# yeyupiaoling/PPASR

Measured on AMD Instinct MI355X. Metric: audio-seconds/s (RTF^-1) Conformer-streaming fbank, batch32 per GPU, ctc_greedy, higher is better.
Workload: dtype f32; 1 GPU; configs[1]: Conformer streaming (configs/conformer.yml), fbank-80, 32 x 10 s utterances per GPU, V=4233, ctc_greedy, features resident in HBM -> token ids + scores on device; global_batch=32, frames=1000, decoder=ctc_greedy, parallelism=utterance-dp1, pipelined=False, gemm=f32

## Files before the change

### ppasr_amd/csrc/capi.hip

```cpp
#include <cxxabi.h>
#include <cstdlib>

#include "capi_internal.h"

namespace ppasr {
thread_local LaunchProf g_launch_prof;
}

static thread_local std::string g_err;
std::string& ppasr_err_slot() { return g_err; }


ppasr_status upload_pe_table(ppasr_model_s* m, BlobMap& sd, const float** pe_dev) {
  const int d = m->desc.output_size > 0 ? m->desc.output_size : kD;
  const int max_len = m->desc.max_len > 0 ? m->desc.max_len : 5000;
  m->desc.max_len = max_len;
  std::vector<float> pe((size_t)max_len * d);
  auto it = sd.find("__pe_table__");
  if (it != sd.end() && it->second.numel() == pe.size()) {
    std::memcpy(pe.data(), it->second.p, pe.size() * sizeof(float));
  } else {
    for (int i = 0; i < d / 2; ++i) {
      float div = expf((float)(2 * i) * (float)(-(std::log(10000.0) / d)));
      for (int pos = 0; pos < max_len; ++pos) {
// ... 290 lines not shown
      }
      const float* ws[3] = {wq, wk, wv};
      UP4(pack_b(d, 3 * d, [&](int k, int n) { return ws[n / d][(size_t)k * d + (n % d)]; }), L.wqkv);
      std::vector<float> bqkv(3 * d);
      std::memcpy(&bqkv[0], bq, d * sizeof(float));
      std::memcpy(&bqkv[d], bk, d * sizeof(float));
      std::memcpy(&bqkv[2 * d], bv, d * sizeof(float));
      UP(bqkv, L.bqkv);
      UP4(pack_b(d, d, [&](int k, int n) { return wo[(size_t)k * d + n]; }), L.wo);
      UP(vec_of(bo, d), L.bo);
      if (rel) {
        UP(vec_of(pu, pbn), L.pos_u);
        UP(vec_of(pv, pbn), L.pos_v);
        const float* bpos_dev = nullptr;
        if (bp) UP(vec_of(bp, d), bpos_dev);
        const float* wpos_dev = nullptr;
        UP(vec_of(wp, (size_t)d * d), wpos_dev);
        void* pt = nullptr;
        HIP_TRY(hipMalloc(&pt, (size_t)max_len * d * sizeof(float)));
        m->allocs.push_back(pt);
        launch_posproj(pe_dev, wpos_dev, bpos_dev, static_cast<float*>(pt), max_len, nullptr, d);
        HIP_TRY(hipGetLastError());
        L.ptab = static_cast<const float*>(pt);
      } else {
        L.pos_u = L.pos_v = L.ptab = m->zero_vec;
      }
      if (go.concat_after) {
        GET(wc, p + "concat_linear.weight", (size_t)2 * d * d);
        GET(bc, p + "concat_linear.bias", d);
        UP4(pack_b(2 * d, d, [&](int k, int n) { return wc[(size_t)k * d + n]; }), m->gen_x[i].wcat);
        UP(vec_of(bc, d), m->gen_x[i].bcat);
      }
    }
    if (go.use_cnn) {
      GET(p1w, p + "conv_module.pointwise_conv1.weight", 2 * d * d);
      GET(p1b, p + "conv_module.pointwise_conv1.bias", 2 * d);
      GET(dww, p + "conv_module.depthwise_conv.weight", d * KSi);
      GET(dwb, p + "conv_module.depthwise_conv.bias", d);
      GET(p2w, p + "conv_module.pointwise_conv2.weight", d * d);
      GET(p2b, p + "conv_module.pointwise_conv2.bias", d);
      UP4(pack_b(d, 2 * d, [&](int k, int n) { return p1w[(size_t)n * d + k]; }), L.pw1);
      std::vector<float> b1p(p1b, p1b + 2 * d), gp(d);
      for (int c = 0; c < d; ++c) gp[c] = p1b[c] * (1.0f / (1.0f + expf(-p1b[c + d])));
      UP(b1p, L.pw1_b);
      UP(gp, L.glu_pad);
      std::vector<float> dwt((size_t)KSi * d);
// ... 464 lines not shown
    bt_off += (n + 15) / 16 * 16;
    p.tab = t;
    return p;
  };
  int Ti = Tp, mul = sub, pstride = 1;
  bool s1_done = false;
  for (int i = 0; i < h->desc.num_blocks; ++i) {
    const LayerW& L = h->layers[i];
    const int Mi = B * Ti;
    const int grp = h->layer_group[i];
    auto fusable = [&](int layer) {
      return h->layer_group[layer] == 1 && h->desc.attention_heads == 4 && !h->taps && fuse_rows(Mi);
    };
    const PadSkip ps = pskip(Ti, mul);
    const int rows = (!h->taps && conv_ffn_16_supported(h->layer_ks[i], Ti)) ? row_block_for(h, B, Ti, mul, ps.slack, skip) : 32;
    const bool r16 = rows == 16 && h->ffn_split < 0;
    const bool fuse_attn = !r16 && fusable(i);
    const int S = r16 ? 1 : ffn_split_for(h, Mi);
    const bool w16 = rows == kW16 && S == 1;
    const PadSkip psb = S == 1 ? with_table(ps, Ti, r16 ? 16 : 32) : ps;
    const bool h3 = h->gemm_mode == PPASR_GEMM_F16X3 && !h->layers_h3.empty() && !r16 && !w16 && S == 1;
    const bool h3s = h->gemm_mode == PPASR_GEMM_F16X3 && !h->layers_h3.empty() && S > 1;
    const LayerW& Lk = (h3 || h3s) ? h->layers_h3[i] : L;
    auto vt_for = [&](bool fused, bool mode) {
      VtOut v = fused ? vt_out : VtOut{};
      v.k_h3 = (fused && mode) ? 1 : 0;
      return v;
    };
    float* partial = y1;
    float* x3 = ctx;
    if (!s1_done) {
      if (S > 1) {
        timed(3, [&] {
          launch_ffn_split(xa, L.ln_mac_g, L.ln_mac_b, Lk.ffm_w1, L.ffm_b1, Lk.ffm_w2, L.ffm_b2, 0.5f, nullptr, nullptr, partial,
                           xb, Mi, n_chunks, S, st, ps, false, h3s);
          launch_ln_qkv(xb, qkv, Lk, Mi, st, ps, nullptr, nullptr, h3s);
        });
      } else if (r16) {
        timed(3, [&] { launch_ffn_qkv_16(xa, xb, qkv, L, Mi, n_chunks, st, psb); });
      } else if (w16) {
        timed(3, [&] { launch_ffn_qkv_w16(xa, xb, qkv, L, Mi, n_chunks, st, psb, fuse_attn ? vt_out : VtOut{}); });
      } else {
        timed(3, [&] { launch_ffn_qkv(xa, xb, qkv, Lk, Mi, n_chunks, st, psb, vt_for(fuse_attn, h3), h3); });
      }
    }
    s1_done = false;
    tap(xb, (size_t)Mi * kD);
    tap(qkv, (size_t)Mi * 3 * kD);
    const int Tt = (Ti + grp - 1) / grp;
    AttnArgs a{qkv, 768, qkv + 256, 768, qkv + 512, 768, Tt, Tt, 0, lens, ctx, L.pos_u, L.pos_v, (h3 && fuse_attn) ? Lk.ptab : L.ptab, pstride,
               mul * grp, Ti, Ti, grp};
    a.pad_skip = skip ? ps.slack + 1 : 0;
    a.vt = vt_out.vt;
    a.vt_stride = vt_out.stride;
    if (fuse_attn) {
      timed(9, [&] { launch_attn_out_glu(a, B, xb, xc, g, Lk, st, h3); });
    } else {
      timed(4, [&] { launch_attention(a, B, h->desc.attention_heads, st); });
      tap(ctx, (size_t)Mi * kD);
      if (r16) timed(5, [&] { launch_out_glu_16(ctx, xb, xc, g, L, lens, Mi, Ti, mul, st, psb); });
      else if (w16) timed(5, [&] { launch_out_glu_w16(ctx, xb, xc, g, L, lens, Mi, Ti, mul, st, psb); });
      else timed(5, [&] { launch_out_glu(ctx, xb, xc, g, nullptr, h3s ? Lk : L, lens, Mi, Ti, mul, st, psb, S > 1 ? xa : nullptr, h3s); });
    }
    tap(xc, (size_t)Mi * kD);
    tap(g, (size_t)Mi * kD);
    if (eff && i == h->desc.stride_layer_idx) {
      const int Ts = (Ti + 1) / 2;
      timed(6, [&] {
        const int Ss = r16 ? 1 : ffn_split_for(h, B * Ts);
        if (Ss > 1) {
          launch_conv_ffn_stride(g, nullptr, xc, xa, h3s ? Lk : L, lens, B, Ti, Ts, n_chunks, h->layer_ks[i], mul * 2, st,
                                 pskip(Ts, mul * 2), h->desc.causal != 0, h3s, ctx);
          launch_ffn_split(ctx, L.ln_ff_g, L.ln_ff_b, Lk.ff_w1, L.ff_b1, Lk.ff_w2, L.ff_b2, 0.5f, L.ln_fin_g, L.ln_fin_b, partial,
                           xa, B * Ts, n_chunks, Ss, st, pskip(Ts, mul * 2), false, h3s);
        } else {
          launch_conv_ffn_stride(g, nullptr, xc, xa, (h3 || h3s) ? Lk : L, lens, B, Ti, Ts, n_chunks, h->layer_ks[i], mul * 2, st,
                                 pskip(Ts, mul * 2), h->desc.causal != 0, h3 || h3s);
        }
      });
      Ti = Ts;
      mul *= 2;
      pstride *= 2;
    } else if (S > 1) {
      timed(6, [&] {
        launch_conv_pre(g, nullptr, xc, x3, Lk, lens, Mi, Ti, h->layer_ks[i], mul, st, h->desc.causal != 0, ps, h3s);
        launch_ffn_split(x3, L.ln_ff_g, L.ln_ff_b, Lk.ff_w1, L.ff_b1, Lk.ff_w2, L.ff_b2, 0.5f, L.ln_fin_g, L.ln_fin_b, partial,
                         xa, Mi, n_chunks, S, st, ps, false, h3s);
      });
    } else {
      const LayerW* next = (i + 1 < h->desc.num_blocks) ? (h3 ? &h->layers_h3[i + 1] : &h->layers[i + 1]) : nullptr;
      timed(next ? 8 : 6, [&] {
        if (r16)
          launch_conv_ffn_16(g, xc, next ? nullptr : xa, L, lens, Mi, Ti, n_chunks, h->layer_ks[i], mul, next, xb, qkv, st,
                             h->desc.causal != 0, psb);
        else if (w16)
          launch_conv_ffn_w16(g, xc, next ? nullptr : xa, L, lens, Mi, Ti, n_chunks, h->layer_ks[i], mul, next, xb, qkv, st,
                              h->desc.causal != 0, psb, (next && fusable(i + 1)) ? vt_out : VtOut{});
        else
          launch_conv_ffn(g, nullptr, xc, (next && !h->taps) ? nullptr : xa, Lk, lens, Mi, Ti, n_chunks, h->layer_ks[i], mul,
                          next, xb, qkv, st, h->desc.causal != 0, psb,
                          vt_for(next && fusable(i + 1), h3), h3);
      });
      s1_done = next != nullptr;
    }
    tap(xa, (size_t)B * Ti * kD);
  }
  const int Mo = B * Ti;
  float* lg = logits ? logits : probs;
  int32_t* fa = frame_argmax ? frame_argmax : reinterpret_cast<int32_t*>(ws + wl.fa);
  float* fp = frame_maxprob ? frame_maxprob : ws + wl.fp;
  timed(7, [&] {
    const bool head_h3 = h->gemm_mode == PPASR_GEMM_F16X3 && h->head_w_h3;
    HeadW hw = h->head;
    if (head_h3) hw.w = h->head_w_h3;
    launch_ctc_head(xa, hw, lg, fa, fp, ws + wl.rmax, ws + wl.rsum, Mo, st, pskip(Ti, mul),
                    wide_slices_for(h, Mo, std::min((hw.n_tiles + 7) / 8, 32)), y1, head_h3);
  });
  if (probs) {
    if (logits)
      HIP_TRY(hipMemcpyAsync(probs, logits, (size_t)Mo * h->head.V * sizeof(float), hipMemcpyDeviceToDevice, st));
    launch_softmax_from_stats(probs, ws + wl.rmax, ws + wl.rsum, Mo, h->head.V, st, pskip(Ti, mul));
  }
  if (skip) launch_zero_pad_rows(probs, logits, fa, fp, lens, B, Ti, mul, h->head.V, st);
  HIP_TRY(hipGetLastError());
// ... 617 lines not shown
```

### ppasr_amd/csrc/conformer_kernels.h

```cpp
#pragma once
#include <hip/hip_runtime.h>
#include <stdint.h>

#include "rowblock.h"

namespace ppasr {

struct LayerW {
  const float *ln_mac_g, *ln_mac_b, *ln_mha_g, *ln_mha_b, *ln_conv_g, *ln_conv_b;
  const float *ln_ff_g, *ln_ff_b, *ln_fin_g, *ln_fin_b, *ln_cm_g, *ln_cm_b;
  float cm_eps;
  const f32x4 *ffm_w1, *ffm_w2, *ff_w1, *ff_w2, *wqkv, *wo, *pw1, *pw2;
  const float *ffm_b1, *ffm_b2, *ff_b1, *ff_b2, *bqkv, *bo, *pw1_b, *pw2_b;
  const float *dw_w;
  const float *dw_b;
  const float *glu_pad;
  const float *pos_u, *pos_v;
  const float *ptab;
};

struct FrontW {
  const float *cmvn_mean, *cmvn_istd;
  const float *conv1_w, *conv1_b;
  const f32x4 *conv2_w;
  const f32x4 *conv2_wp = nullptr;
  const float *conv2_b;
  int conv2_k = 3, conv2_s = 2;
  const f32x4 *conv3_w = nullptr;
  const float *conv3_b = nullptr;
  const f32x4 *embed_w;
  const float *embed_b;
};

struct HeadW {
  const float *ln_g, *ln_b;
  const f32x4 *w;
  const float *b;
  int V, n_tiles;
};

struct SessDesc {
// ... 6 lines not shown
struct AttnArgs {
  const float* q;
  int q_stride;
  const float* k;
  int k_stride;
  const float* v;
  int v_stride;
  int T1, T2;
  int pos0;
  const int64_t* lens;
  float* ctx;
  const float *pos_u, *pos_v;
  const float* ptab;
  int pos_stride;
  int mask_mul;
  int q_frames, kv_frames;
  int group;
  const SessDesc* sess;
  long long sess_stride;
  int pad_skip;
  const float* vt = nullptr;
  int vt_stride = 0;
  int dm = 256;
};
struct VtOut {
  float* vt = nullptr;
  int stride = 0;
  int k_h3 = 0;
};

constexpr size_t kLdsExclusive = 82 * 1024;
size_t ragged_lds(size_t lds, const PadSkip& ps, int n_blocks);

bool launch_attention_t(const AttnArgs& a, int B, int H, hipStream_t st);
hipError_t configure_attention_kernels();

void launch_block_table(const PadSkip& ps, int M, int R, int* tab, hipStream_t st);

bool conv2_quad_supported(const FrontW& fw);
bool conv12_supported(const FrontW& fw, int F, int F2);
void launch_conv12(const float* feats, const FrontW& fw, float* y2, int B, int T, int F, int Tp, int F2, hipStream_t st,
                   const PadSkip& ps_frames, int* tile_scratch);
void launch_conv2_quad(const float* y1, const FrontW& fw, float* y2, int B, int T1, int F1, int Tp, int F2, hipStream_t st,
                       const PadSkip& ps_frames, int* tile_scratch);
hipError_t configure_front_fused_kernels();

void launch_ffn_qkv_16(const float* x_in, float* x1, float* qkv, const LayerW& w, int M, int n_chunks, hipStream_t st,
                       const PadSkip& ps);
void launch_out_glu_16(const float* ctx, const float* x1, float* x2, float* g, const LayerW& w, const int64_t* lens, int M,
                       int Tp, int mask_mul, hipStream_t st, const PadSkip& ps);
void launch_out_glu_split_16(const float* ctx, const float* x1, float* x2, float* g, float* xhat, const LayerW& w,
// ... 1 lines not shown
                             float* hist = nullptr, int lo = 0);
void launch_shift_caches(float* kc, float* vc, long long layer_stride, int D, int n_layers, int from_full, int keep_full,
                         int from_half, int keep_half, unsigned long long half_mask, hipStream_t st);
void launch_oproj_ln_16(const float* ctx, const float* x1, float* x2_sink, float* xhat_out, const LayerW& w, int M,
                        hipStream_t st, const PadSkip& ps = PadSkip{});
void launch_pw1_glu_cols_16(const float* x, float* g, const LayerW& w, int M, hipStream_t st, float* hist = nullptr, int lo = 0,
                            const float* hist_scale = nullptr, const float* hist_bias = nullptr, const PadSkip& ps = PadSkip{},
                            const int64_t* lens = nullptr, int Tp = 1, int mask_mul = 1);
bool conv_ffn_16_supported(int ksize, int Tp);
void launch_conv_ffn_16(const float* g, const float* x2, float* x_out, const LayerW& w, const int64_t* lens, int M, int Tp,
                        int n_chunks, int ksize, int mask_mul, const LayerW* next, float* x1_next, float* qkv_next,
                        hipStream_t st, bool causal, const PadSkip& ps);
void launch_ffn_qkv_w16(const float* x_in, float* x1, float* qkv, const LayerW& w, int M, int n_chunks, hipStream_t st,
                        const PadSkip& ps, VtOut vt);
void launch_out_glu_w16(const float* ctx, const float* x1, float* x2, float* g, const LayerW& w, const int64_t* lens, int M,
                        int Tp, int mask_mul, hipStream_t st, const PadSkip& ps);
void launch_conv_ffn_w16(const float* g, const float* x2, float* x_out, const LayerW& w, const int64_t* lens, int M, int Tp,
                         int n_chunks, int ksize, int mask_mul, const LayerW* next, float* x1_next, float* qkv_next,
                         hipStream_t st, bool causal, const PadSkip& ps, VtOut vt_next);
hipError_t configure_conformer_t_kernels();

void launch_posproj(const float* pe, const float* wpos , const float* bpos_or_null, float* ptab,
                    int max_len, hipStream_t st, int d = 256);
void launch_conv1(const float* feats, const FrontW& fw, float* y1, int B, int T, int F, int T1, int F1, hipStream_t st,
                  const PadSkip& ps = PadSkip{}, int channels = 256);
void launch_conv_stage(const float* y_in, const f32x4* w, const float* bias, float* y_out, int B, int T_in, int F_in,
                       int T_out, int F_out, int k, int s, hipStream_t st, const PadSkip& ps_frames = PadSkip{},
                       int channels = 256, int* tile_scratch = nullptr,
                       bool h3 = false,
                       float* part = nullptr, size_t part_floats = 0);
size_t conv_stage_part_floats(int M, int channels = 256);
size_t conv_stage_part_reserve(int M);
void launch_conv2(const float* y1, const FrontW& fw, float* y2, int B, int T1, int F1, int Tp, int F2, hipStream_t st,
                  const PadSkip& ps = PadSkip{}, int* tile_scratch = nullptr, const f32x4* w_h3 = nullptr, float* part = nullptr,
                  size_t part_floats = 0);
void launch_embed(const float* y2, const FrontW& fw, float* x0, int M, int K, float xscale, bool scale_before_bias,
                  hipStream_t st, const PadSkip& ps = PadSkip{}, int k_slices = 1, float* part = nullptr,
                  const f32x4* w_h3 = nullptr);
void launch_dense(const float* a, int lda, const f32x4* w, const float* bias, float* out, int M, int K, int n_cols_padded,
                  int ldc, int n_valid, hipStream_t st, float scale = 1.0f, float* part = nullptr, size_t part_floats = 0);
void launch_ffn_qkv(const float* x_in, float* x1, float* qkv, const LayerW& w, int M, int n_chunks, hipStream_t st,
                    const PadSkip& ps = PadSkip{}, VtOut vt = VtOut{}, bool h3 = false);
void launch_repack_h3(const f32x4* src, f32x4* dst, int n_tiles, int G, unsigned int* ovf, hipStream_t st);
inline bool conv_ffn_h3_supported(int ksize) { return ksize == 15 || ksize == 7; }
void launch_split_rows_h3(const float* src, float* dst, long long n_rows, unsigned int* ovf, hipStream_t st);
unsigned int* conformer_h3_ovf_counter();
// ... 87 lines not shown
```

### ppasr_amd/csrc/conformer_kernels.hip

```cpp
#include <cstdlib>

#include "conformer_kernels.h"
#include "launch.h"
#include "phases.h"
#include "h3.h"

#include <math.h>

namespace ppasr {
#ifdef PPASR_PHASE_TS
}
extern "C" __attribute__((visibility("default"))) int ppasr_debug_read_phase_ts(long long* out) {
  return (int)hipMemcpyFromSymbol(out, HIP_SYMBOL(ppasr::g_phase_ts), sizeof(long long) * 128);
}
extern "C" __attribute__((visibility("default"))) int ppasr_debug_read_wave_ts(long long* out) {
  return (int)hipMemcpyFromSymbol(out, HIP_SYMBOL(ppasr::g_wave_ts), sizeof(long long) * 512);
}
extern "C" __attribute__((visibility("default"))) int ppasr_debug_read_wg_ts(long long* out) {
  return (int)hipMemcpyFromSymbol(out, HIP_SYMBOL(ppasr::g_wg_ts), sizeof(long long) * 2 * 1024);
}
namespace ppasr {
#endif


// ... 40 lines not shown

template <bool H3 = false>
__device__ __forceinline__ void ffn_qkv_body(float* bufX, float* bufA, float* bufH, float* __restrict__ x1,
                                             float* __restrict__ qkv, const LayerW& w, int r0, int valid, int n_chunks,
                                             BRing<1>& ring, VtOut vt = VtOut{}) {
  const int lane = lane_id(), wave = wave_id();
  rb_layernorm(bufX, bufA, kLda, kRows, w.ln_mac_g, w.ln_mac_b, 1e-5f);
  __syncthreads();
  PPASR_TS(8);
  f32x16 acc2[1][1];
  acc_zero(acc2);
  const f32x4* wq = w.wqkv + (size_t)wave * kTs256;
  if constexpr (H3) ffn_phase_h3(bufA, w.ffm_w1, w.ffm_b1, w.ffm_w2, n_chunks, wq, ring, acc2);
  else ffn_phase<true>(bufA, bufH, w.ffm_w1, w.ffm_b1, w.ffm_w2, n_chunks, wq, ring, acc2);
  PPASR_TS(9);
  residual_epilogue_t(bufX, acc2, w.ffm_b2, 0.5f);
  __syncthreads();
  PPASR_TS(10);
  rb_store_rows(x1 + (size_t)r0 * kD, bufX, kLda, kRows, valid);
  rb_layernorm(bufX, bufA, kLda, kRows, w.ln_mha_g, w.ln_mha_b, 1e-5f);
  __syncthreads();
  if constexpr (H3) h3_planes_from_tile(bufA, reinterpret_cast<_Float16*>(bufA));
  PPASR_TS(11);
  f32x16 tile[3][1][1];
  bool qk_bad = false;
  const int cq = wave * 32 + 4 * (lane >> 5);
  float* qrow = (lane & 31) < valid ? qkv + (size_t)(r0 + (lane & 31)) * 768 + cq : nullptr;
  f32x4 qb[2][4];
#pragma unroll
  for (int c = 0; c < 2; ++c)
#pragma unroll
    for (int q = 0; q < 4; ++q) qb[c][q] = *reinterpret_cast<const f32x4*>(w.bqkv + c * 256 + cq + 8 * q);
#pragma unroll
  for (int c = 0; c < 3; ++c) {
    acc_zero(tile[c]);
    const f32x4* seg = w.wqkv + (size_t)(c * 8 + wave) * kTs256;
    const f32x4* nseg = c < 2 ? seg + 8 * kTs256 : nullptr;
    if constexpr (H3) {
      const _Float16* pa = reinterpret_cast<const _Float16*>(bufA);
      if (c < 2)
        rb_gemm_h3(pa, seg, nseg, ring, tile[c][0][0]);
      else
        rb_gemm_h3_rows<1, 16, QkStoreTailH3>(pa, kLdh, kPlaneH, seg, nseg, ring, tile[c],
                                              QkStoreTailH3{tile[0][0][0], tile[1][0][0], qrow, qb, vt.k_h3 != 0, qk_bad, cq});
    } else if (c == 0) {
      rb_gemm<1, 1, kG256, kPF, NoSide, true>(bufA, kLda, seg, 0, nseg, 0, ring, tile[c]);
    } else if (c == 1) {
      rb_gemm<1, 1, kG256, kPF, QkvStoreSide, true>(bufA, kLda, seg, 0, nseg, 0, ring, tile[c],
                                                    QkvStoreSide{tile[0][0][0], qrow, qb[0]});
    } else {
      rb_gemm<1, 1, kG256, kPF, QkvStoreSide, false>(bufA, kLda, seg, 0, nseg, 0, ring, tile[c],
                                                     QkvStoreSide{tile[1][0][0], qrow ? qrow + 256 : nullptr, qb[1]});
    }
    PPASR_TS(12 + c);
  }
  if constexpr (H3) h3_note(qk_bad);
  if (vt.vt) {
    const float bv = w.bqkv[2 * 256 + wave * 32 + (lane & 31)];
    float* dst = vt.vt + ((size_t)wave * (vt.stride >> 3) + (r0 >> 3)) * 256 + 4 * lane;
    if constexpr (H3) tile[2][0][0] *= kH3Inv;
#pragma unroll
    for (int i = 0; i < 4; ++i) {
      const f32x16& t = tile[2][0][0];
      *reinterpret_cast<f32x4*>(dst + i * 256) = f32x4{t[4 * i] + bv, t[4 * i + 1] + bv, t[4 * i + 2] + bv, t[4 * i + 3] + bv};
    }
  } else {
    const int col = 2 * 256 + wave * 32 + (lane & 31);
    const float bv = w.bqkv[col];
    if constexpr (H3) tile[2][0][0] *= kH3Inv;
#pragma unroll
    for (int r = 0; r < 16; ++r) {
      int row = acc_row(r, lane);
      if (row < valid) qkv[(size_t)(r0 + row) * 768 + col] = tile[2][0][0][r] + bv;
    }
  }
}
// ... 212 lines not shown
    launch_out_glu_split_16(ctx, x1, x2, g, xh, w, lens, M, Tp, mask_mul, st, ps, move ? hm->hist : nullptr, move ? hm->lo : 0);
    if (move) hm->done = true;
    return;
  }
  const dim3 grid((M + kRows - 1) / kRows);
  if (h3)
    PPASR_LAUNCH(k_out_glu<true>, grid, dim3(kThreads), kLdsOutGlu + 512, st, ctx, x1, x2, g, xh, w, lens, M, Tp, mask_mul, ps,
                 split_xhat ? 1 : 0);
  else
    PPASR_LAUNCH(k_out_glu<false>, grid, dim3(kThreads), kLdsOutGlu, st, ctx, x1, x2, g, xh, w, lens, M, Tp, mask_mul, ps,
                 split_xhat ? 1 : 0);
  if (split_xhat) {
    if (h3)
      PPASR_LAUNCH(k_pw1_glu_cols<true>, dim3(grid.x, 2), dim3(kThreads), kLdsPw1Cols + 512, st, xh, g, w, M, ps);
    else
      PPASR_LAUNCH(k_pw1_glu_cols<false>, dim3(grid.x, 2), dim3(kThreads), kLdsPw1Cols, st, xh, g, w, M, ps);
  }
}

constexpr int kPLd = 68;
constexpr int kPTile = 32 * kPLd;
constexpr int kFusedAttnFloats = kWaves * kPTile + kWaves * 64 + kRows * kLda;
static_assert(2 * kRows * kLda <= kWaves * kPTile + kWaves * 64, "bufX/bufA alias the attention scratch");
static_assert(kRows * kLda + 128 + 4 * kPTile <= kWaves * kPTile, "Q'_v (fp16 x3: its planes, 512 B longer) and the four merge tiles fit in front of Stat");
static_assert(kH3TileBytes <= kRows * kLda * 4 + 512, "fp16 x3: the Q'_u planes at bufC run 512 B past it (the launch asks for them)");
static_assert(kRows * kLda * 4 + kH3TileBytes <= kWaves * kPTile * 4, "fp16 x3: operand planes at bufA stay in front of Stat");
static_assert(kFusedAttnFloats * 4 <= 160 * 1024, "LDS budget");
template <bool H3>
__device__ __forceinline__ void attn_out_glu_body(const AttnArgs& a, int B, const float* __restrict__ x1, float* __restrict__ x2,
                                                  float* __restrict__ g, const LayerW& w) {
  extern __shared__ __attribute__((aligned(16))) float smem[];
  float* Ps = smem;
  float* Stat = Ps + kWaves * kPTile;
  float* bufC = Stat + kWaves * 64;
  float* bufX = smem;
  float* bufA = bufX + kRows * kLda;
  const int lane = lane_id(), wave = wave_id();
  const int h = wave >> 1, khalf = wave & 1;
  const int nq = (a.T1 + 31) / 32;
  const int slot = blockIdx.x >> 3;
  const int b = (slot / nq) * 8 + (blockIdx.x & 7);
  const int q0 = (slot % nq) * 32;
  if (b >= B) return;
  const int T = a.T1;
  const int valid = min(32, T - q0);
  const float* __restrict__ qb = a.q + (size_t)b * T * a.q_stride;
  const float* __restrict__ kbp = a.k + (size_t)b * a.T2 * a.k_stride;
  const float* __restrict__ vbp = a.v + (size_t)b * a.T2 * a.v_stride;
  const float* __restrict__ ptab = a.ptab + (size_t)a.pos0 * kD;
  const int pstride = a.pos_stride;
  const int64_t len_b = a.lens ? a.lens[b] : (int64_t)a.mask_mul * a.T2;
  int T2 = a.T2;
  if (a.pad_skip > 0 && a.lens) {
    const int64_t lb = len_b > 0 ? len_b : 0;
    const int64_t n_valid = (lb + a.mask_mul - 1) / a.mask_mul;
    if (q0 >= min((int64_t)T, n_valid + (a.pad_skip - 1))) return;
    T2 = (int)max((int64_t)1, min((int64_t)T2, n_valid));
  }
  float* QV = Ps;
  float* P = Ps + kRows * kLda + (H3 ? 128 : 0) + (wave >> 1) * kPTile;
  BRing<1> ring;
  const f32x4* seg_o = w.wo + (size_t)wave * kTs256;
  const f32x4* seg_val = w.pw1 + (size_t)wave * kTs256;
  const f32x4* seg_gate = w.pw1 + (size_t)(8 + wave) * kTs256;
  const int hh = lane >> 5, l31 = lane & 31;
  constexpr int NG = 16, PF = 4;
  PPASR_TS(32);
  PPASR_WG_TS(512 + 0);

  const int mrow0 = b * T;
  const int shift = mrow0 & 7;
  int kv_end = (int)min((int64_t)T2, max((int64_t)0, (len_b + a.mask_mul - 1) / a.mask_mul));
  const int U = kv_end > 0 ? kv_end + shift : 0;
  constexpr float kScale = 0.125f * 1.4426950408889634f * (H3 ? 1.0f / (kH3Sa * kH3Sa) : 1.0f);
  const __amdgpu_buffer_rsrc_t rs_k = wstream_rsrc(kbp + h * (H3 ? 32 : 64)), rs_p = wstream_rsrc(ptab + h * (H3 ? 32 : 64)),
                               rs_v = wstream_rsrc(a.vt + ((size_t)(2 * h) * (a.vt_stride >> 3) + ((mrow0 - shift) >> 3)) * 256);
  const int voff_v = lane * 16;
  const int kstride_b = a.k_stride * 4, pstride_b = pstride * kD * 4;
  int vk[2], vp[2];
  auto key_offsets = [&](int u0) {
#pragma unroll
    for (int t = 0; t < 2; ++t) {
      const int key = min(max(u0 - shift + 32 * t + l31, 0), kv_end - 1);
      vk[t] = key * kstride_b + 16 * hh;
      vp[t] = key * pstride_b + 16 * hh;
    }
  };
  auto kfrag = [&](int t, int gk) -> f32x4 {
    return gk < 8 ? wstream_load(rs_k, vk[t], gk * 32) : wstream_load(rs_p, vp[t], (gk - 8) * 32);
  };
  constexpr int NKB = H3 ? 4 : 2;
  f32x4 kq[NKB][4][2];
  auto load_sg = [&](int buf, int sg) {
#pragma unroll
    for (int i = 0; i < 4; ++i) {
      if constexpr (H3) {
        const int soff = (sg & 1) * 512 + 32 * i;
        kq[buf][i][0] = sg < 2 ? wstream_load(rs_k, vk[0], soff) : wstream_load(rs_p, vp[0], soff);
        kq[buf][i][1] = sg < 2 ? wstream_load(rs_k, vk[1], soff) : wstream_load(rs_p, vp[1], soff);
      } else {
        kq[buf][i][0] = kfrag(0, 4 * sg + i);
        kq[buf][i][1] = kfrag(1, 4 * sg + i);
      }
    }
  };
  auto prime_k = [&](int u0) {
    key_offsets(u0);
    load_sg(0, 0);
    if constexpr (H3) load_sg(1, 1);
  };

  {
    const f32x4 pu = *reinterpret_cast<const f32x4*>(a.pos_u + 4 * lane), pv = *reinterpret_cast<const f32x4*>(a.pos_v + 4 * lane);
    bool bad = false;
    for (int row = wave; row < kRows; row += kWaves) {
      f32x4 v = {0.f, 0.f, 0.f, 0.f};
      if (row < valid) v = *reinterpret_cast<const f32x4*>(qb + (size_t)(q0 + row) * a.q_stride + 4 * lane);
      if constexpr (H3) {
        f16x4 hi, lo;
        h3_split4((v + pu) * kH3Sa, hi, lo, bad);
        _Float16* pu_pl = reinterpret_cast<_Float16*>(bufC) + row * kLdh + 4 * lane;
        *reinterpret_cast<f16x4*>(pu_pl) = hi;
        *reinterpret_cast<f16x4*>(pu_pl + kPlaneH) = lo;
        h3_split4((v + pv) * kH3Sa, hi, lo, bad);
        _Float16* pv_pl = reinterpret_cast<_Float16*>(QV) + row * kLdh + 4 * lane;
        *reinterpret_cast<f16x4*>(pv_pl) = hi;
        *reinterpret_cast<f16x4*>(pv_pl + kPlaneH) = lo;
      } else {
        *reinterpret_cast<f32x4*>(bufC + row * kLda + 4 * lane) = v + pu;
        *reinterpret_cast<f32x4*>(QV + row * kLda + 4 * lane) = v + pv;
      }
    }
    if constexpr (H3) h3_note(bad);
    __syncthreads();
  }
  const float* qfrag_u = bufC + l31 * kLda + h * 64 + 4 * hh;
  const float* qfrag_v = QV + l31 * kLda + h * 64 + 4 * hh;
  auto qfrag = [&](int gk) -> f32x4 {
    return *reinterpret_cast<const f32x4*>(gk < 8 ? qfrag_u + 8 * gk : qfrag_v + 8 * (gk - 8));
  };
  PPASR_TS(33);
  if (khalf * 128 < U) prime_k(khalf * 128);
  f32x16 acc_o[2];
#pragma unroll
  for (int t = 0; t < 2; ++t)
#pragma unroll
    for (int r = 0; r < 16; ++r) acc_o[t][r] = 0.f;
  float m_run = -INFINITY, l_run = 0.f;
  bool first = true;

  const int nkb = (U + 255) / 256;
  for (int kb = 0; kb < nkb; ++kb) {
    for (int sb = 0; sb < 2; ++sb) {
      const int u0 = kb * 256 + khalf * 128 + sb * 64;
      if (u0 >= U) break;
      int u_next = sb == 0 ? u0 + 64 : (kb + 1) * 256 + khalf * 128;
      if (u_next >= U) u_next = (sb == 0 && (kb + 1) * 256 + khalf * 128 < U) ? (kb + 1) * 256 + khalf * 128 : -1;
      const bool edge = (u0 < shift) || (u0 + 64 > U);
      if (kb == 0) PPASR_WAVE_TS(16 + 4 * sb);
      const int soff_v = (u0 >> 3) * 1024, soff_v1 = soff_v + (a.vt_stride >> 3) * 1024;
      auto vload = [&](int q, int ct) -> f32x4 { return wstream_load(rs_v, voff_v, (ct ? soff_v1 : soff_v) + q * 1024); };
      constexpr int PQ = 8;
      f32x4 ringv[PQ][2];
      auto prime_v = [&]() {
#pragma unroll
        for (int q = 0; q < PQ; ++q) {
          ringv[q][0] = vload(q, 0);
          ringv[q][1] = vload(q, 1);
        }
      };
      f32x16 acc_s[2];
#pragma unroll
      for (int t = 0; t < 2; ++t)
#pragma unroll
        for (int r = 0; r < 16; ++r) acc_s[t][r] = 0.f;
      if constexpr (H3) {
        const _Float16* qu = reinterpret_cast<const _Float16*>(bufC) + l31 * kLdh + h * 64 + 8 * hh;
        const _Float16* qv = reinterpret_cast<const _Float16*>(QV) + l31 * kLdh + h * 64 + 8 * hh;
        load_sg(2, 2);
        load_sg(3, 3);
#pragma unroll
        for (int sg = 0; sg < 4; ++sg) {
          const _Float16* qp = sg < 2 ? qu : qv;
#pragma unroll
          for (int i = 0; i < 4; ++i) {
            const f16x8 qh = *reinterpret_cast<const f16x8*>(qp + 16 * i);
            const f16x8 k0 = __builtin_bit_cast(f16x8, kq[sg][i][0]), k1 = __builtin_bit_cast(f16x8, kq[sg][i][1]);
            if ((sg & 1) == 0) {
              const f16x8 ql = *reinterpret_cast<const f16x8*>(qp + kPlaneH + 16 * i);
              acc_s[0] = __builtin_amdgcn_mfma_f32_32x32x16_f16(k0, ql, acc_s[0], 0, 0, 0);
              acc_s[1] = __builtin_amdgcn_mfma_f32_32x32x16_f16(k1, ql, acc_s[1], 0, 0, 0);
            }
            acc_s[0] = __builtin_amdgcn_mfma_f32_32x32x16_f16(k0, qh, acc_s[0], 0, 0, 0);
            acc_s[1] = __builtin_amdgcn_mfma_f32_32x32x16_f16(k1, qh, acc_s[1], 0, 0, 0);
            __builtin_amdgcn_sched_barrier(0);
          }
        }
      } else {
        f32x4 q_cur = qfrag(0), q_nxt = q_cur;
#pragma unroll
        for (int sg = 0; sg < 4; ++sg) {
          if (sg + 1 < 4) load_sg((sg + 1) & 1, sg + 1);
#pragma unroll
          for (int i = 0; i < 4; ++i) {
            const int gk = 4 * sg + i;
            if (gk + 1 < NG) q_nxt = qfrag(gk + 1);
            const f32x4 k0 = kq[sg & 1][i][0], k1 = kq[sg & 1][i][1];
#pragma unroll
            for (int j = 0; j < 4; ++j) {
              acc_s[0] = __builtin_amdgcn_mfma_f32_32x32x2f32(k0[j], q_cur[j], acc_s[0], 0, 0, 0);
              acc_s[1] = __builtin_amdgcn_mfma_f32_32x32x2f32(k1[j], q_cur[j], acc_s[1], 0, 0, 0);
            }
            q_cur = q_nxt;
            __builtin_amdgcn_sched_barrier(0);
          }
        }
      }
      if (kb == 0) PPASR_WAVE_TS(17 + 4 * sb);
      prime_v();
      if (edge) {
        const int lo = shift - u0 - 4 * hh, hi = U - u0 - 4 * hh;
        if (u0 < shift) {
#pragma unroll
          for (int r = 0; r < 4; ++r)
            if (r < lo) acc_s[0][r] = -INFINITY;
        }
        if (u0 + 64 > U) {
#pragma unroll
          for (int t = 0; t < 2; ++t)
#pragma unroll
// ... 497 lines not shown
```

### ppasr_amd/csrc/conformer_kernels_t.hip

```cpp
#include "conformer_kernels.h"
#include "launch.h"
#include "phases_t.h"

namespace ppasr {

#ifdef PPASR_PHASE_TS
}
extern "C" __attribute__((visibility("default"))) int ppasr_debug_read_phase_ts_t(long long* out) {
  return (int)hipMemcpyFromSymbol(out, HIP_SYMBOL(ppasr::g_phase_ts), sizeof(long long) * 128);
}
namespace ppasr {
#endif

template <int R>
__device__ __forceinline__ void ffn_qkv_body_t(float* bufX, float* bufA, float* bufH, float* __restrict__ x1,
                                               float* __restrict__ qkv, const LayerW& w, int r0, int valid, int n_chunks,
                                               typename RBT<R>::Ring& ring, VtOut vt = VtOut{}) {
  using T = RBT<R>;
  const LaneT<R> L;
  rbt_layernorm<R>(bufX, bufA, w.ln_mac_g, w.ln_mac_b, 1e-5f);
  __syncthreads();
  PPASR_TS(8);
  typename T::Acc acc2;
  T::zero(acc2);
  ffn_phase_t<R>(bufA, bufH, w.ffm_w1, w.ffm_b1, w.ffm_w2, n_chunks, w.wqkv + (size_t)L.tile() * kTs256, ring, acc2);
  PPASR_TS(9);
  residual_epilogue_q<R>(bufX, acc2, w.ffm_b2, 0.5f);
  __syncthreads();
  PPASR_TS(10);
  rbt_store_rows<R>(x1 + (size_t)r0 * kD, bufX, valid);
  rbt_layernorm<R>(bufX, bufA, w.ln_mha_g, w.ln_mha_b, 1e-5f);
  __syncthreads();
  PPASR_TS(11);
  qkv_phase_t<R>(bufA, qkv, w.wqkv, w.bqkv, r0, valid, ring, vt.vt, vt.stride);
  PPASR_TS(14);
}

template <int R>
__global__ __launch_bounds__(RBT<R>::THREADS) void k_ffn_qkv_t(const float* __restrict__ x_in, float* __restrict__ x1,
                                                               float* __restrict__ qkv, LayerW w, int M, int n_chunks,
                                                               PadSkip ps, VtOut vt) {
  using T = RBT<R>;
  extern __shared__ __attribute__((aligned(16))) float smem[];
  const int blk = pad_block_of(ps, T::ROWS, M);
  if (blk < 0) return;
  float* bufX = smem;
  float* bufA = bufX + T::ROWS * kLda;
  float* bufH = bufA + T::ROWS * kLda;
  const int r0 = blk * T::ROWS;
  const int valid = min(T::ROWS, M - r0);
  typename T::Ring ring;
  rbt_prime(ring, w.ffm_w1 + (size_t)T::tile(wave_id()) * kTs256);
  rbt_load_rows<R>(bufX, x_in + (size_t)r0 * kD, valid);
  ffn_qkv_body_t<R>(bufX, bufA, bufH, x1, qkv, w, r0, valid, n_chunks, ring, vt);
}

template <int R>
// ... 331 lines not shown
```

### ppasr_amd/csrc/front_kernels.hip

```cpp
#include <algorithm>
#include <cstdlib>

#include "conformer_kernels.h"
#include "launch.h"
#include "phases.h"
#include "h3.h"

#include <math.h>

namespace ppasr {
#ifdef PPASR_PHASE_TS
}
extern "C" __attribute__((visibility("default"))) int ppasr_debug_read_wave_ts_front(long long* out) {
  return (int)hipMemcpyFromSymbol(out, HIP_SYMBOL(ppasr::g_wave_ts), sizeof(long long) * 512);
}
namespace ppasr {
#endif

__global__ void k_posproj(const float* __restrict__ pe, const float* __restrict__ wpos,
                          const float* __restrict__ bpos, float* __restrict__ ptab, int max_len, int d) {
  int pos = blockIdx.x;
  int n = threadIdx.x;
  __shared__ float row[1024];
  row[n] = pe[(size_t)pos * d + n];
// ... 450 lines not shown
unsigned int* front_h3_ovf_counter() { return h3_ovf_counter(); }

hipError_t configure_front_kernels() {
  hipError_t e = hipSuccess;
#define SET_LDS(fn, bytes)                                                                                     \
  e = hipFuncSetAttribute(reinterpret_cast<const void*>(fn), hipFuncAttributeMaxDynamicSharedMemorySize, (int)(bytes)); \
  if (e != hipSuccess) return e;
  SET_LDS(k_conv_stage_h3<4>, 2 * 2 * 128 * 136 * sizeof(_Float16));
  SET_LDS(k_conv_stage_h3<3>, 2 * 2 * 96 * 136 * sizeof(_Float16));
  SET_LDS(k_conv_stage_h3<2>, 2 * 2 * 64 * 136 * sizeof(_Float16));
  SET_LDS(k_conv_stage_h3<1>, 2 * 2 * 32 * 136 * sizeof(_Float16));
  SET_LDS((k_gemm_stream<4, 128, true, false, Conv2Src>), 2 * 128 * 132 * sizeof(float));
  SET_LDS((k_gemm_stream<3, 128, true, false, Conv2Src>), 2 * 96 * 132 * sizeof(float));
  SET_LDS((k_gemm_stream<2, 128, true, false, Conv2Src>), 2 * 64 * 132 * sizeof(float));
  SET_LDS((k_gemm_stream<1, 128, true, false, Conv2Src>), 2 * 32 * 132 * sizeof(float));
  SET_LDS(k_embed_h3<false>, kLdsExclusive);
  SET_LDS(k_embed_h3<true>, kLdsExclusive);
  SET_LDS((k_gemm_stream<1, 256, false, false, DenseSrc>), kLdsExclusive);
  SET_LDS((k_gemm_stream<1, 256, false, true, DenseSrc>), kLdsExclusive);
#undef SET_LDS
  return hipSuccess;
}

}
```

### ppasr_amd/csrc/phases.h

```cpp
#pragma once
#include "rowblock.h"

namespace ppasr {

struct SwishSide {
  const f32x16& acc;
  float* dst;
  const f32x4 (&bias)[4];
  mutable f32x2 lo;
  __device__ __forceinline__ void operator()(int g) const {
    const int q = g >> 3;
    if ((g & 7) == 0) lo = swish2(f32x2{acc[4 * q] + bias[q][0], acc[4 * q + 1] + bias[q][1]});
    if ((g & 7) == 4) {
      const f32x2 hi = swish2(f32x2{acc[4 * q + 2] + bias[q][2], acc[4 * q + 3] + bias[q][3]});
      *reinterpret_cast<f32x4*>(dst + 8 * q) = f32x4{lo[0], lo[1], hi[0], hi[1]};
    }
  }
};

template <bool T2 = false>
__device__ __forceinline__ void ffn_phase(const float* bufA, float* bufH, const f32x4* __restrict__ w1,
                                          const float* __restrict__ b1, const f32x4* __restrict__ w2, int n_chunks,
                                          const f32x4* __restrict__ after, BRing<1>& ring, f32x16 (&acc2)[1][1],
                                          int c0 = 0, int n_total = -1) {
// ... 159 lines not shown
#pragma unroll
    for (int i = 0; i < RW; ++i) acc[i] = bias;
#pragma unroll
    for (int q = 0; q < NW; ++q) {
      const int tt = tqp - left + q;
      const f32x4 xq = (tt >= 0 && tt < Tp) ? x[q] : gp;
#pragma unroll
      for (int i = 0; i < RW; ++i) {
        const int j = q - i;
        if (j >= 0 && j < KS) acc[i] += wt[j] * xq;
      }
    }
#pragma unroll
    for (int i = 0; i < RW; ++i)
      if (npass == 1 || (tqp + i >= 0 && tqp + i < Tp)) out[i] = acc[i];
  }
  const f32x4 gam = *reinterpret_cast<const f32x4*>(ln_g + 4 * lane);
  const f32x4 bet = *reinterpret_cast<const f32x4*>(ln_b + 4 * lane);
  ln_rows_inreg<true, RW>(out, gam, bet, ln_eps);
#pragma unroll
  for (int i = 0; i < RW; ++i) *reinterpret_cast<f32x4*>(bufA + (q0 + i) * kLda + 4 * lane) = out[i];
}

}
```

### ppasr_amd/csrc/phases_t.h

```cpp
#pragma once
#include "phases.h"
#include "rbt.h"

namespace ppasr {

template <int R>
struct LaneT {
  int lane, wave;
  __device__ __forceinline__ LaneT() : lane(lane_id()), wave(wave_id()) {}
  __device__ __forceinline__ int row(int q) const { return RBT<R>::row(q, lane); }
  __device__ __forceinline__ int col(int q) const { return RBT<R>::col(q, lane, wave); }
  __device__ __forceinline__ int off(int q) const { return row(q) * kLda + col(q); }
  __device__ __forceinline__ int tile() const { return RBT<R>::tile(wave); }
  __device__ __forceinline__ int quads_ok(int valid) const {
    int n = 0;
#pragma unroll
    for (int q = 0; q < RBT<R>::NQ; ++q) n += row(q) < valid ? 1 : 0;
    return n;
  }
};

template <int R>
__device__ __forceinline__ void rbt_load_rows(float* dst, const float* __restrict__ src, int valid) {
  const int lane = lane_id();
// ... 126 lines not shown
  }
}

template <int R>
struct QuadStoreSide {
  const typename RBT<R>::Acc& acc;
  float* out;
  int qstep;
  int n_ok;
  const f32x4 (&bias)[RBT<R>::NQ];
  __device__ __forceinline__ void operator()(int g) const {
    constexpr int STEP = 32 / RBT<R>::NQ;
    const int q = g / STEP;
    if (g % STEP == STEP / 2 && q < n_ok) {
      const f32x4 v = RBT<R>::quad(acc, q);
      *reinterpret_cast<f32x4*>(out + q * qstep) = f32x4{v[0] + bias[q][0], v[1] + bias[q][1], v[2] + bias[q][2], v[3] + bias[q][3]};
    }
  }
};

template <int R>
__device__ __forceinline__ void qkv_phase_t(const float* bufX, float* __restrict__ qkv, const f32x4* __restrict__ wqkv,
                                            const float* __restrict__ bqkv, int r0, int valid, typename RBT<R>::Ring& ring,
                                            float* __restrict__ vt = nullptr, int vt_stride = 0) {
  using T = RBT<R>;
  const LaneT<R> L;
  float* q0 = qkv + (size_t)(r0 + L.row(0)) * 768 + L.col(0);
  const int qs = T::qstep(768), n_ok = L.quads_ok(valid);
  f32x4 qb[3][T::NQ];
#pragma unroll
  for (int c = 0; c < 3; ++c)
#pragma unroll
    for (int q = 0; q < T::NQ; ++q) qb[c][q] = *reinterpret_cast<const f32x4*>(bqkv + c * 256 + L.col(q));
  typename T::Acc tile[3];
#pragma unroll
  for (int c = 0; c < 3; ++c) {
    T::zero(tile[c]);
    const f32x4* seg = wqkv + (size_t)(c * 8 + L.tile()) * kTs256;
    const f32x4* nseg = c < 2 ? seg + 8 * kTs256 : nullptr;
    if (c == 0) {
      rbt_gemm<kG256>(bufX, kLda, seg, nseg, ring, tile[c]);
    } else {
      const QuadStoreSide<R> store{tile[c - 1], q0 + (c - 1) * 256, qs, n_ok, qb[c - 1]};
      if constexpr (R == kW16) {
        if (c == 2 && vt) rbt_gemm<kG256, QuadStoreSide<R>, false>(bufX, kLda, seg, nseg, ring, tile[c], store);
        else rbt_gemm<kG256>(bufX, kLda, seg, nseg, ring, tile[c], store);
      } else {
        rbt_gemm<kG256>(bufX, kLda, seg, nseg, ring, tile[c], store);
      }
    }
  }
  if constexpr (R == kW16) {
    if (vt) {
      const int c32 = 16 * (L.wave & 1) + (L.lane & 15), kq = L.lane >> 4;
      const float bv = bqkv[512 + 16 * L.wave + (L.lane & 15)];
      float* dst = vt + ((size_t)(L.wave >> 1) * (vt_stride >> 3) + (r0 >> 3) + (kq >> 1)) * 256 + 4 * (c32 + 32 * (kq & 1));
// ... 98 lines not shown
```

Measured before the change: 57610 audio-s/s.

## Fold positional term into K and a precomputed per-head bias table for rel-pos attention

Rewrites the relative-position attention score (q+u)·k + (q+v)·p as (q+u)·(k+p) + (v−u)·p. The positional vector p is added to K at QKV projection time, and the (v−u)·p term is precomputed once per layer into a per-head table, dtab. In the fp32 fused attention path this halves the score GEMM reduction (NG 16→8), drops the Q'_v staging buffer and the positional-table streaming, and initialises the accumulators from dtab staged in LDS. The cost is an extra bias load per K row in the QKV phase and one table per layer, plus a numerics change from the reassociated sum.

New measurement: 58250 audio-s/s (median of 6 runs). 1.01x the previous value.

```diff
diff --git a/ppasr_amd/csrc/capi.hip b/ppasr_amd/csrc/capi.hip
--- a/ppasr_amd/csrc/capi.hip
+++ b/ppasr_amd/csrc/capi.hip
@@ -336,6 +336,14 @@
         launch_posproj(pe_dev, wpos_dev, bpos_dev, static_cast<float*>(pt), max_len, nullptr, d);
         HIP_TRY(hipGetLastError());
         L.ptab = static_cast<const float*>(pt);
+        if (!grouped && d == kD && desc->attention_heads == 4) {
+          void* dt = nullptr;
+          HIP_TRY(hipMalloc(&dt, (size_t)4 * max_len * sizeof(float)));
+          m->allocs.push_back(dt);
+          launch_pos_dtab(L.ptab, L.pos_u, L.pos_v, static_cast<float*>(dt), max_len, nullptr);
+          HIP_TRY(hipGetLastError());
+          L.dtab = static_cast<const float*>(dt);
+        }
       } else {
         L.pos_u = L.pos_v = L.ptab = m->zero_vec;
       }
@@ -846,9 +854,14 @@
     const bool h3 = h->gemm_mode == PPASR_GEMM_F16X3 && !h->layers_h3.empty() && !r16 && !w16 && S == 1;
     const bool h3s = h->gemm_mode == PPASR_GEMM_F16X3 && !h->layers_h3.empty() && S > 1;
     const LayerW& Lk = (h3 || h3s) ? h->layers_h3[i] : L;
-    auto vt_for = [&](bool fused, bool mode) {
+    auto vt_for = [&](bool fused, bool mode, int layer) {
       VtOut v = fused ? vt_out : VtOut{};
       v.k_h3 = (fused && mode) ? 1 : 0;
+      if (fused && !mode && h->layers[layer].dtab) {
+        v.kpos = h->layers[layer].ptab;
+        v.kpos_stride = pstride * kD;
+        v.Ti = Ti;
+      }
       return v;
     };
     float* partial = y1;
@@ -863,9 +876,9 @@
       } else if (r16) {
         timed(3, [&] { launch_ffn_qkv_16(xa, xb, qkv, L, Mi, n_chunks, st, psb); });
       } else if (w16) {
-        timed(3, [&] { launch_ffn_qkv_w16(xa, xb, qkv, L, Mi, n_chunks, st, psb, fuse_attn ? vt_out : VtOut{}); });
+        timed(3, [&] { launch_ffn_qkv_w16(xa, xb, qkv, L, Mi, n_chunks, st, psb, vt_for(fuse_attn, false, i)); });
       } else {
-        timed(3, [&] { launch_ffn_qkv(xa, xb, qkv, Lk, Mi, n_chunks, st, psb, vt_for(fuse_attn, h3), h3); });
+        timed(3, [&] { launch_ffn_qkv(xa, xb, qkv, Lk, Mi, n_chunks, st, psb, vt_for(fuse_attn, h3, i), h3); });
       }
     }
     s1_done = false;
@@ -877,6 +890,10 @@
     a.pad_skip = skip ? ps.slack + 1 : 0;
     a.vt = vt_out.vt;
     a.vt_stride = vt_out.stride;
+    if (fuse_attn && !h3) {
+      a.dtab = L.dtab;
+      a.dtab_len = h->desc.max_len;
+    }
     if (fuse_attn) {
       timed(9, [&] { launch_attn_out_glu(a, B, xb, xc, g, Lk, st, h3); });
     } else {
@@ -919,11 +936,11 @@
                              h->desc.causal != 0, psb);
         else if (w16)
           launch_conv_ffn_w16(g, xc, next ? nullptr : xa, L, lens, Mi, Ti, n_chunks, h->layer_ks[i], mul, next, xb, qkv, st,
-                              h->desc.causal != 0, psb, (next && fusable(i + 1)) ? vt_out : VtOut{});
+                              h->desc.causal != 0, psb, vt_for(next && fusable(i + 1), false, i + 1));
         else
           launch_conv_ffn(g, nullptr, xc, (next && !h->taps) ? nullptr : xa, Lk, lens, Mi, Ti, n_chunks, h->layer_ks[i], mul,
                           next, xb, qkv, st, h->desc.causal != 0, psb,
-                          vt_for(next && fusable(i + 1), h3), h3);
+                          vt_for(next && fusable(i + 1), h3, next ? i + 1 : i), h3);
       });
       s1_done = next != nullptr;
     }
diff --git a/ppasr_amd/csrc/conformer_kernels.h b/ppasr_amd/csrc/conformer_kernels.h
--- a/ppasr_amd/csrc/conformer_kernels.h
+++ b/ppasr_amd/csrc/conformer_kernels.h
@@ -17,6 +17,7 @@
   const float *glu_pad;
   const float *pos_u, *pos_v;
   const float *ptab;
+  const float *dtab = nullptr;
 };
 
 struct FrontW {
@@ -69,11 +70,16 @@
   const float* vt = nullptr;
   int vt_stride = 0;
   int dm = 256;
+  const float* dtab = nullptr;
+  int dtab_len = 0;
 };
 struct VtOut {
   float* vt = nullptr;
   int stride = 0;
   int k_h3 = 0;
+  const float* kpos = nullptr;
+  int kpos_stride = 0;
+  int Ti = 1;
 };
 
 constexpr size_t kLdsExclusive = 82 * 1024;
@@ -121,6 +127,7 @@
 
 void launch_posproj(const float* pe, const float* wpos , const float* bpos_or_null, float* ptab,
                     int max_len, hipStream_t st, int d = 256);
+void launch_pos_dtab(const float* ptab, const float* pos_u, const float* pos_v, float* dtab, int max_len, hipStream_t st);
 void launch_conv1(const float* feats, const FrontW& fw, float* y1, int B, int T, int F, int T1, int F1, hipStream_t st,
                   const PadSkip& ps = PadSkip{}, int channels = 256);
 void launch_conv_stage(const float* y_in, const f32x4* w, const float* bias, float* y_out, int B, int T_in, int F_in,
diff --git a/ppasr_amd/csrc/conformer_kernels.hip b/ppasr_amd/csrc/conformer_kernels.hip
--- a/ppasr_amd/csrc/conformer_kernels.hip
+++ b/ppasr_amd/csrc/conformer_kernels.hip
@@ -86,15 +86,14 @@
   __syncthreads();
   if constexpr (H3) h3_planes_from_tile(bufA, reinterpret_cast<_Float16*>(bufA));
   PPASR_TS(11);
-  f32x16 tile[3][1][1];
-  bool qk_bad = false;
+  f32x16 tile[3][1][1]; bool qk_bad = false;
   const int cq = wave * 32 + 4 * (lane >> 5);
   float* qrow = (lane & 31) < valid ? qkv + (size_t)(r0 + (lane & 31)) * 768 + cq : nullptr;
-  f32x4 qb[2][4];
-#pragma unroll
-  for (int c = 0; c < 2; ++c)
-#pragma unroll
-    for (int q = 0; q < 4; ++q) qb[c][q] = *reinterpret_cast<const f32x4*>(w.bqkv + c * 256 + cq + 8 * q);
+  f32x4 qb[2][4], kp[4];
+#pragma unroll
+  for (int c = 0; c < 3; ++c)
+#pragma unroll
+    for (int q = 0; q < 4; ++q) (c < 2 ? qb[c][q] : kp[q]) = qkv_bias_quad<H3>(w.bqkv, vt, c, r0 + (lane & 31), cq + 8 * q);
 #pragma unroll
   for (int c = 0; c < 3; ++c) {
     acc_zero(tile[c]);
@@ -116,6 +115,7 @@
       rb_gemm<1, 1, kG256, kPF, QkvStoreSide, false>(bufA, kLda, seg, 0, nseg, 0, ring, tile[c],
                                                      QkvStoreSide{tile[1][0][0], qrow ? qrow + 256 : nullptr, qb[1]});
     }
+    if (c == 0) qkv_kpos_add<H3>(qb[1], kp, vt);
     PPASR_TS(12 + c);
   }
   if constexpr (H3) h3_note(qk_bad);
@@ -374,7 +374,7 @@
 constexpr int kPTile = 32 * kPLd;
 constexpr int kFusedAttnFloats = kWaves * kPTile + kWaves * 64 + kRows * kLda;
 static_assert(2 * kRows * kLda <= kWaves * kPTile + kWaves * 64, "bufX/bufA alias the attention scratch");
-static_assert(kRows * kLda + 128 + 4 * kPTile <= kWaves * kPTile, "Q'_v (fp16 x3: its planes, 512 B longer) and the four merge tiles fit in front of Stat");
+static_assert(kRows * kLda + 128 + 4 * kPTile <= kWaves * kPTile, "the d rows (fp16 x3: the Q'_v planes, 512 B longer) and the four merge tiles fit in front of Stat");
 static_assert(kH3TileBytes <= kRows * kLda * 4 + 512, "fp16 x3: the Q'_u planes at bufC run 512 B past it (the launch asks for them)");
 static_assert(kRows * kLda * 4 + kH3TileBytes <= kWaves * kPTile * 4, "fp16 x3: operand planes at bufA stay in front of Stat");
 static_assert(kFusedAttnFloats * 4 <= 160 * 1024, "LDS budget");
@@ -416,7 +416,7 @@
   const f32x4* seg_val = w.pw1 + (size_t)wave * kTs256;
   const f32x4* seg_gate = w.pw1 + (size_t)(8 + wave) * kTs256;
   const int hh = lane >> 5, l31 = lane & 31;
-  constexpr int NG = 16, PF = 4;
+  constexpr int NG = H3 ? 16 : 8;
   PPASR_TS(32);
   PPASR_WG_TS(512 + 0);
 
@@ -435,11 +435,8 @@
     for (int t = 0; t < 2; ++t) {
       const int key = min(max(u0 - shift + 32 * t + l31, 0), kv_end - 1);
       vk[t] = key * kstride_b + 16 * hh;
-      vp[t] = key * pstride_b + 16 * hh;
-    }
-  };
-  auto kfrag = [&](int t, int gk) -> f32x4 {
-    return gk < 8 ? wstream_load(rs_k, vk[t], gk * 32) : wstream_load(rs_p, vp[t], (gk - 8) * 32);
+      if constexpr (H3) vp[t] = key * pstride_b + 16 * hh;
+    }
   };
   constexpr int NKB = H3 ? 4 : 2;
   f32x4 kq[NKB][4][2];
@@ -451,8 +448,8 @@
         kq[buf][i][0] = sg < 2 ? wstream_load(rs_k, vk[0], soff) : wstream_load(rs_p, vp[0], soff);
         kq[buf][i][1] = sg < 2 ? wstream_load(rs_k, vk[1], soff) : wstream_load(rs_p, vp[1], soff);
       } else {
-        kq[buf][i][0] = kfrag(0, 4 * sg + i);
-        kq[buf][i][1] = kfrag(1, 4 * sg + i);
+        kq[buf][i][0] = wstream_load(rs_k, vk[0], (4 * sg + i) * 32);
+        kq[buf][i][1] = wstream_load(rs_k, vk[1], (4 * sg + i) * 32);
       }
     }
   };
@@ -462,7 +459,9 @@
     if constexpr (H3) load_sg(1, 1);
   };
 
+  const float* __restrict__ dtab = a.dtab ? a.dtab + (size_t)h * a.dtab_len + a.pos0 : nullptr;
   {
+    if constexpr (!H3) attn_stage_d(Ps + h * kDRow, dtab, khalf * 64 + lane, shift, U <= kDRow ? U : 0, pstride);
     const f32x4 pu = *reinterpret_cast<const f32x4*>(a.pos_u + 4 * lane), pv = *reinterpret_cast<const f32x4*>(a.pos_v + 4 * lane);
     bool bad = false;
     for (int row = wave; row < kRows; row += kWaves) {
@@ -480,17 +479,13 @@
         *reinterpret_cast<f16x4*>(pv_pl + kPlaneH) = lo;
       } else {
         *reinterpret_cast<f32x4*>(bufC + row * kLda + 4 * lane) = v + pu;
-        *reinterpret_cast<f32x4*>(QV + row * kLda + 4 * lane) = v + pv;
       }
     }
     if constexpr (H3) h3_note(bad);
     __syncthreads();
   }
   const float* qfrag_u = bufC + l31 * kLda + h * 64 + 4 * hh;
-  const float* qfrag_v = QV + l31 * kLda + h * 64 + 4 * hh;
-  auto qfrag = [&](int gk) -> f32x4 {
-    return *reinterpret_cast<const f32x4*>(gk < 8 ? qfrag_u + 8 * gk : qfrag_v + 8 * (gk - 8));
-  };
+  auto qfrag = [&](int gk) -> f32x4 { return *reinterpret_cast<const f32x4*>(qfrag_u + 8 * gk); };
   PPASR_TS(33);
   if (khalf * 128 < U) prime_k(khalf * 128);
   f32x16 acc_o[2];
@@ -522,10 +517,14 @@
         }
       };
       f32x16 acc_s[2];
-#pragma unroll
-      for (int t = 0; t < 2; ++t)
-#pragma unroll
-        for (int r = 0; r < 16; ++r) acc_s[t][r] = 0.f;
+      if constexpr (H3) {
+#pragma unroll
+        for (int t = 0; t < 2; ++t)
+#pragma unroll
+          for (int r = 0; r < 16; ++r) acc_s[t][r] = 0.f;
+      } else {
+        attn_score_init(acc_s, U <= kDRow ? Ps + h * kDRow + u0 + 4 * hh : nullptr, dtab, u0 - shift + 4 * hh, kv_end, pstride);
+      }
       if constexpr (H3) {
         const _Float16* qu = reinterpret_cast<const _Float16*>(bufC) + l31 * kLdh + h * 64 + 8 * hh;
         const _Float16* qv = reinterpret_cast<const _Float16*>(QV) + l31 * kLdh + h * 64 + 8 * hh;
@@ -551,13 +550,13 @@
       } else {
         f32x4 q_cur = qfrag(0), q_nxt = q_cur;
 #pragma unroll
-        for (int sg = 0; sg < 4; ++sg) {
-          if (sg + 1 < 4) load_sg((sg + 1) & 1, sg + 1);
+        for (int sg = 0; sg < 2; ++sg) {
+          if (sg == 0) load_sg(1, 1);
 #pragma unroll
           for (int i = 0; i < 4; ++i) {
             const int gk = 4 * sg + i;
             if (gk + 1 < NG) q_nxt = qfrag(gk + 1);
-            const f32x4 k0 = kq[sg & 1][i][0], k1 = kq[sg & 1][i][1];
+            const f32x4 k0 = kq[sg][i][0], k1 = kq[sg][i][1];
 #pragma unroll
             for (int j = 0; j < 4; ++j) {
               acc_s[0] = __builtin_amdgcn_mfma_f32_32x32x2f32(k0[j], q_cur[j], acc_s[0], 0, 0, 0);
diff --git a/ppasr_amd/csrc/conformer_kernels_t.hip b/ppasr_amd/csrc/conformer_kernels_t.hip
--- a/ppasr_amd/csrc/conformer_kernels_t.hip
+++ b/ppasr_amd/csrc/conformer_kernels_t.hip
@@ -32,7 +32,7 @@
   rbt_layernorm<R>(bufX, bufA, w.ln_mha_g, w.ln_mha_b, 1e-5f);
   __syncthreads();
   PPASR_TS(11);
-  qkv_phase_t<R>(bufA, qkv, w.wqkv, w.bqkv, r0, valid, ring, vt.vt, vt.stride);
+  qkv_phase_t<R>(bufA, qkv, w.wqkv, w.bqkv, r0, valid, ring, vt.vt, vt.stride, vt.kpos, vt.kpos_stride, vt.Ti);
   PPASR_TS(14);
 }
 
diff --git a/ppasr_amd/csrc/front_kernels.hip b/ppasr_amd/csrc/front_kernels.hip
--- a/ppasr_amd/csrc/front_kernels.hip
+++ b/ppasr_amd/csrc/front_kernels.hip
@@ -496,4 +496,17 @@
   return hipSuccess;
 }
 
-}
+__global__ __launch_bounds__(256) void k_pos_dtab(const float* __restrict__ ptab, const float* __restrict__ pos_u,
+                                                  const float* __restrict__ pos_v, float* __restrict__ dtab, int max_len) {
+  const int t = blockIdx.x * 256 + threadIdx.x, h = blockIdx.y;
+  if (t >= max_len) return;
+  double acc = 0.0;
+  for (int c = 0; c < 64; ++c)
+    acc += ((double)pos_v[64 * h + c] - (double)pos_u[64 * h + c]) * (double)ptab[(size_t)t * 256 + 64 * h + c];
+  dtab[(size_t)h * max_len + t] = (float)acc;
+}
+void launch_pos_dtab(const float* ptab, const float* pos_u, const float* pos_v, float* dtab, int max_len, hipStream_t st) {
+  PPASR_LAUNCH(k_pos_dtab, dim3((max_len + 255) / 256, 4), dim3(256), 0, st, ptab, pos_u, pos_v, dtab, max_len);
+}
+
+}
diff --git a/ppasr_amd/csrc/phases.h b/ppasr_amd/csrc/phases.h
--- a/ppasr_amd/csrc/phases.h
+++ b/ppasr_amd/csrc/phases.h
@@ -1,4 +1,5 @@
 #pragma once
+#include "conformer_kernels.h"
 #include "rowblock.h"
 
 namespace ppasr {
@@ -205,4 +206,46 @@
   for (int i = 0; i < RW; ++i) *reinterpret_cast<f32x4*>(bufA + (q0 + i) * kLda + 4 * lane) = out[i];
 }
 
-}
+template <bool H3>
+__device__ __forceinline__ f32x4 qkv_bias_quad(const float* __restrict__ bqkv, const VtOut& vt, int c, int m, int col) {
+  if (c < 2) return *reinterpret_cast<const f32x4*>(bqkv + c * 256 + col);
+  if constexpr (!H3) {
+    if (vt.kpos) return *reinterpret_cast<const f32x4*>(vt.kpos + (size_t)(m - m / vt.Ti * vt.Ti) * vt.kpos_stride + col);
+  }
+  return f32x4{0.f, 0.f, 0.f, 0.f};
+}
+template <bool H3>
+__device__ __forceinline__ void qkv_kpos_add(f32x4 (&bk)[4], const f32x4 (&kp)[4], const VtOut& vt) {
+  if constexpr (!H3) {
+    if (vt.kpos) {
+#pragma unroll
+      for (int q = 0; q < 4; ++q) bk[q] += kp[q];
+    }
+  }
+}
+constexpr int kDRow = 2048;
+static_assert(4 * kDRow <= kRows * kLda, "the four heads' d rows fit in front of the merge tiles");
+__device__ __forceinline__ void attn_stage_d(float* row, const float* __restrict__ dtab, int t128, int shift, int U, int pstride) {
+  for (int u = t128; u < ((U + 63) & ~63); u += 128)
+    row[u] = (dtab && u >= shift && u < U) ? dtab[(size_t)(u - shift) * pstride] : 0.f;
+}
+__device__ __forceinline__ void attn_score_init(f32x16 (&acc_s)[2], const float* dl, const float* __restrict__ dtab, int key0,
+                                                int kv_end, int pstride) {
+#pragma unroll
+  for (int t = 0; t < 2; ++t)
+#pragma unroll
+    for (int i = 0; i < 4; ++i) {
+      f32x4 dq;
+      if (dl) {
+        dq = *reinterpret_cast<const f32x4*>(dl + 32 * t + 8 * i);
+      } else {
+#pragma unroll
+        for (int j = 0; j < 4; ++j)
+          dq[j] = dtab ? dtab[(size_t)min(max(key0 + 32 * t + 8 * i + j, 0), kv_end - 1) * pstride] : 0.f;
+      }
+#pragma unroll
+      for (int j = 0; j < 4; ++j) acc_s[t][4 * i + j] = dq[j];
+    }
+}
+
+}
diff --git a/ppasr_amd/csrc/phases_t.h b/ppasr_amd/csrc/phases_t.h
--- a/ppasr_amd/csrc/phases_t.h
+++ b/ppasr_amd/csrc/phases_t.h
@@ -172,7 +172,8 @@
 template <int R>
 __device__ __forceinline__ void qkv_phase_t(const float* bufX, float* __restrict__ qkv, const f32x4* __restrict__ wqkv,
                                             const float* __restrict__ bqkv, int r0, int valid, typename RBT<R>::Ring& ring,
-                                            float* __restrict__ vt = nullptr, int vt_stride = 0) {
+                                            float* __restrict__ vt = nullptr, int vt_stride = 0,
+                                            const float* __restrict__ kpos = nullptr, int kpos_stride = 0, int Ti = 1) {
   using T = RBT<R>;
   const LaneT<R> L;
   float* q0 = qkv + (size_t)(r0 + L.row(0)) * 768 + L.col(0);
@@ -182,6 +183,13 @@
   for (int c = 0; c < 3; ++c)
 #pragma unroll
     for (int q = 0; q < T::NQ; ++q) qb[c][q] = *reinterpret_cast<const f32x4*>(bqkv + c * 256 + L.col(q));
+  if (kpos) {
+#pragma unroll
+    for (int q = 0; q < T::NQ; ++q) {
+      const int m = r0 + L.row(q);
+      qb[1][q] += *reinterpret_cast<const f32x4*>(kpos + (size_t)(m - m / Ti * Ti) * kpos_stride + L.col(q));
+    }
+  }
   typename T::Acc tile[3];
 #pragma unroll
   for (int c = 0; c < 3; ++c) {
```
